# yukiteruono/pbsim3

Measured on AMD Instinct MI355X. Metric: simulated bases/sec, higher is better.
Workload: dtype u8

## Files before the change

### pbsim3_amd/csrc/ctx.h

```cpp
#pragma once
#include <hip/hip_runtime.h>
#include <limits.h>
#include <stdio.h>
#include <stdlib.h>
#include <stdint.h>

#include <algorithm>
#include <condition_variable>
#include <functional>
#include <memory>
#include <mutex>
#include <string>
#include <vector>

#include "../../include/pbsim3_amd.h"
#include "host_tables.h"
#include "kernels.h"

namespace pbsim {
extern thread_local std::string g_err;
int fail(const std::string &m);
}


// ... 33 lines not shown
  }
  template <class T>
  T *as() const {
    return reinterpret_cast<T *>(p);
  }
};

struct HostBuf {
  void *p = nullptr;
  size_t bytes = 0;
  ~HostBuf() {
    if (p) (void)hipHostFree(p);
  }
  hipError_t ensure(size_t n) {
    if (n <= bytes) return hipSuccess;
    if (p) (void)hipHostFree(p);
    p = nullptr;
    bytes = 0;
    size_t want = std::max<size_t>(n + n / 8 + 4096, 1u << 20);
    hipError_t e = hipHostMalloc(&p, want, hipHostMallocDefault);
    if (e != hipSuccess) {
      p = nullptr;
      return e;
    }
    bytes = want;
    return hipSuccess;
  }
};

using namespace pbsim;

constexpr int kMaxSlots = 6;
constexpr int kPipelineDepth = 2;
static_assert(kPipelineDepth >= 1 && kPipelineDepth <= kMaxSlots, "the pipeline's slots are the first of kMaxSlots");

constexpr size_t kScratchSlack = 64u << 10;
constexpr double kSinkBatchBases = 5.0e9;

constexpr int kDfBuffers = 5;
struct DfLane {
  DevBuf d_df_status, d_df_ctl;
  uint32_t epoch = 0;
  DevBuf d_df_dense[kDfBuffers];
  DevBuf d_df_code;
  HostBuf h_df_total, h_df_out[kDfBuffers];
  hipStream_t stream = nullptr;
  hipStream_t copy_stream = nullptr;
  bool own_streams = false;
  hipStream_t own[2] = {nullptr, nullptr};
  bool pre_valid = false, pre_own_staging = false, pre_elsewhere = false;
  const uint8_t *pre_text = nullptr;
  int64_t pre_n = 0;
  int pre_count = 0;
  hipStream_t lane_stream = nullptr;
  hipEvent_t ev_pre = nullptr;
  hipEvent_t ev_hand = nullptr;
  bool hand_open = false;
  hipEvent_t ev_df[kDfBuffers] = {}, ev_cp[kDfBuffers] = {};
  hipEvent_t ev_k0[kDfBuffers] = {}, ev_k1[kDfBuffers] = {};
  std::vector<std::unique_ptr<HostBuf>> arena_blocks;
  std::vector<size_t> arena_fill;
  std::vector<char> arena_touched;
  std::vector<int> arena_idle;
  std::vector<std::pair<const char *, int64_t>> arena_segs;
  size_t arena_bytes() const {
    size_t n = 0;
    for (const auto &b : arena_blocks) n += b->bytes;
    return n;
  }
  void arena_reset() {
    std::fill(arena_fill.begin(), arena_fill.end(), 0);
    arena_segs.clear();
  }
  char *arena_reserve(int64_t n, size_t max_bytes) {
    static const size_t kBlock = getenv("PBSIM_PINNED_BLOCK_KB") && atoll(getenv("PBSIM_PINNED_BLOCK_KB")) > 0
                                     ? (size_t)atoll(getenv("PBSIM_PINNED_BLOCK_KB")) << 10 : (size_t)256u << 20;
    const size_t need = ((size_t)n + 63) & ~(size_t)63;
    for (size_t i = 0; i < arena_blocks.size(); i++) {
      HostBuf &b = *arena_blocks[i];
      if (arena_fill[i] + need <= b.bytes) {
        char *p = (char *)b.p + arena_fill[i];
        arena_fill[i] += need;
        arena_touched[i] = 1;
        arena_segs.emplace_back(p, n);
        return p;
      }
    }
    const size_t want = std::max(kBlock, need);
    if (max_bytes && arena_bytes() + want > max_bytes) return nullptr;
    if (getenv("PBSIM_TRACE")) fprintf(stderr, "[pbsim arena] new block of %zu MB (lane holds %zu MB in %zu blocks)\n", want >> 20, arena_bytes() >> 20, arena_blocks.size());
    arena_blocks.emplace_back(new HostBuf);
    arena_fill.push_back(0);
    arena_touched.push_back(1);
    arena_idle.push_back(0);
    if (arena_blocks.back()->ensure(want) != hipSuccess) {
      arena_blocks.pop_back();
      arena_fill.pop_back();
      arena_touched.pop_back();
      arena_idle.pop_back();
      return nullptr;
    }
    arena_fill.back() = need;
    arena_segs.emplace_back((char *)arena_blocks.back()->p, n);
    return (char *)arena_blocks.back()->p;
  }
  static constexpr int kArenaIdleJobs = 16;
// ... 236 lines not shown
```

### pbsim3_amd/csrc/deflate_host.cpp

```cpp
#include <hip/hip_runtime.h>
#include <limits.h>
#include <math.h>
#include <stdio.h>
#include <stdlib.h>
#include <string.h>

#include <algorithm>
#include <chrono>
#include <functional>
#include <memory>
#include <string>
#include <thread>
#include <vector>

#include "ctx.h"
#include "engine_internal.h"
#include "unit_io.h"

extern "C" {

extern "C++" {
namespace {

int ensure_deflate_tables(pbsim_ctx *c) {
  if (c->d_df_tables.p) return PBSIM_SUCCEEDED;
  std::vector<uint32_t> t(1024 + 256);
  deflate_host_tables(t.data(), t.data() + 1024);
  if (!upload(c->d_df_tables, t.data(), t.size() * 4, c->stream)) return PBSIM_FAILED;
  HIP_OK(hipStreamSynchronize(c->stream));
  return PBSIM_SUCCEEDED;
}

struct DfGeom {
  int64_t piece, max_ch, n_pieces;
  int ahead, nbuf;
  int64_t off(int64_t j) const { return j * piece; }
  int64_t len(int64_t j, int64_t n) const { return std::min(piece, n - off(j)); }
};
DfGeom df_geom(int64_t n) {
  constexpr int64_t piece_chunks = DF_PIECE_CHUNKS;
  constexpr int kDfAhead = 4;
  static_assert(kDfAhead >= 1 && kDfAhead <= kDfBuffers - 1, "ahead + 1 dense buffers are in use");
  DfGeom g;
  g.piece = piece_chunks * DF_CHUNK;
  g.max_ch = std::min<int64_t>(piece_chunks, (n + DF_CHUNK - 1) / DF_CHUNK);
  g.n_pieces = (n + g.piece - 1) / g.piece;
  g.ahead = kDfAhead;
  g.nbuf = g.ahead + 1;
  return g;
}

int df_launch_piece(pbsim_ctx *c, DfLane &sl, const DfGeom &g, const uint8_t *d_text, int64_t n, int64_t j, bool wait_buffer,
                    bool own_staging, unsigned long long *d_prof) {
  const int b = (int)(j % g.nbuf);
  const int64_t off = g.off(j), len = g.len(j, n);
  const uint32_t *tab = c->d_df_tables.as<uint32_t>();
  int64_t *h_total = reinterpret_cast<int64_t *>(sl.h_df_total.p);
  HIP_OK(sl.d_df_dense[b].ensure((size_t)g.max_ch * DF_SLOT + 64, true));
  if (own_staging) HIP_OK(sl.h_df_out[b].ensure((size_t)g.max_ch * DF_SLOT + 64));
  if (wait_buffer) HIP_OK(hipStreamWaitEvent(sl.stream, sl.ev_cp[b], 0));
  uint8_t *dense = sl.d_df_dense[b].as<uint8_t>();
  if (((sl.epoch + 1) & 0x3fffffffu) == 0) {
    HIP_OK(hipMemsetAsync(sl.d_df_status.p, 0, sl.d_df_status.bytes, sl.stream));
    sl.epoch++;
  }
  launch_deflate(d_text + off, len, sl.d_df_status.as<uint64_t>(), sl.d_df_ctl.p, ++sl.epoch, dense, tab, tab + 1024,
                 sl.d_df_code.p, sl.stream, d_prof, sl.ev_k0[b], sl.ev_k1[b]);
  HIP_OK(hipGetLastError());
  HIP_OK(hipMemcpyAsync(&h_total[2 * b], sl.d_df_ctl.p, DF_CTL_BYTES, hipMemcpyDeviceToHost, sl.stream));
  HIP_OK(hipEventRecord(sl.ev_df[b], sl.stream));
  return PBSIM_SUCCEEDED;
}

int df_begin(pbsim_ctx *c, DfLane &sl, const uint8_t *d_text, int64_t n, bool own_staging, hipStream_t launch_stream) {
  if (!ensure_deflate_tables(c)) return PBSIM_FAILED;
  const DfGeom g = df_geom(n);
  const size_t status_bytes_was = sl.d_df_status.bytes;
  HIP_OK(sl.d_df_status.ensure((size_t)(g.piece / DF_CHUNK) * 8));
  HIP_OK(sl.d_df_ctl.ensure(DF_CTL_BYTES));
  HIP_OK(sl.h_df_total.ensure(DF_CTL_BYTES * kDfBuffers));
  HIP_OK(sl.d_df_code.ensure(DF_TABLE_BYTES + 288 * 4));
  int lane_index = 0;
  for (Slot &slot : c->slots)
    if (&slot.df[1] == &sl) lane_index = 1;
  hipStream_t lane_streams[2];
  if (sl.own_streams) {
    for (int i = 0; i < 2; i++)
      if (!sl.own[i]) HIP_OK(hipStreamCreateWithFlags(&sl.own[i], hipStreamNonBlocking));
    lane_streams[0] = sl.own[0];
    lane_streams[1] = sl.own[1];
  } else {
    for (int i = 0; i < 2; i++)
      if (!c->df_streams[lane_index][i]) HIP_OK(hipStreamCreateWithFlags(&c->df_streams[lane_index][i], hipStreamNonBlocking));
    lane_streams[0] = c->df_streams[lane_index][0];
    lane_streams[1] = c->df_streams[lane_index][1];
  }
  sl.lane_stream = lane_streams[0];
  sl.stream = launch_stream ? launch_stream : lane_streams[0];
  sl.copy_stream = lane_streams[1];
  if (sl.d_df_status.bytes != status_bytes_was) HIP_OK(hipMemsetAsync(sl.d_df_status.p, 0, sl.d_df_status.bytes, sl.stream));
  launch_deflate_table(d_text, n, reinterpret_cast<uint32_t *>(sl.d_df_code.as<uint8_t>() + DF_TABLE_BYTES), sl.d_df_code.p, sl.stream);
  if (!sl.ev_df[0]) {
    for (int i = 0; i < kDfBuffers; i++) {
      HIP_OK(hipEventCreateWithFlags(&sl.ev_df[i], hipEventDisableTiming));
      HIP_OK(hipEventCreateWithFlags(&sl.ev_cp[i], hipEventDisableTiming));
      HIP_OK(hipEventCreate(&sl.ev_k0[i]));
      HIP_OK(hipEventCreate(&sl.ev_k1[i]));
    }
  }
  unsigned long long *d_prof = nullptr;
  if (getenv("PBSIM_DEFLATE_PROF")) {
    HIP_OK(c->d_df_prof.ensure(128));
    HIP_OK(hipMemsetAsync(c->d_df_prof.p, 0, 128, sl.stream));
    d_prof = c->d_df_prof.as<unsigned long long>();
  }
  const int64_t first = std::min<int64_t>(launch_stream ? 1 : g.ahead, g.n_pieces);
  for (int64_t j = 0; j < first; j++)
    if (!df_launch_piece(c, sl, g, d_text, n, j, false, own_staging, d_prof)) return PBSIM_FAILED;
  sl.pre_count = (int)first;
  sl.pre_text = d_text;
  sl.pre_n = n;
  sl.pre_own_staging = own_staging;
  sl.pre_valid = true;
  sl.pre_elsewhere = launch_stream != nullptr;
  if (launch_stream) {
    if (!sl.ev_pre) HIP_OK(hipEventCreateWithFlags(&sl.ev_pre, hipEventDisableTiming));
    HIP_OK(hipEventRecord(sl.ev_pre, launch_stream));
  }
  return PBSIM_SUCCEEDED;
}

template <class F>
int deflate_stream(pbsim_ctx *c, DfLane &sl, const uint8_t *d_text, int64_t n, F &&consume,
                   const std::function<char *(int64_t)> *place = nullptr, const std::function<bool()> *tail_hook = nullptr) {
  if (n <= 0) return PBSIM_SUCCEEDED;
  const bool prelaunched = sl.pre_valid && sl.pre_text == d_text && sl.pre_n == n && sl.pre_own_staging == (place == nullptr);
  sl.pre_valid = false;
  const bool handed = prelaunched && sl.hand_open;
  if (!prelaunched && !pbsim::deflate_settle(sl)) return PBSIM_FAILED;
  if (!prelaunched && !df_begin(c, sl, d_text, n, place == nullptr, nullptr)) return PBSIM_FAILED;
  sl.pre_valid = false;
  if (handed && getenv("PBSIM_TRACE"))
    fprintf(stderr, "[deflate] lane call of %.1f MB found its head handed off (%d pieces launched behind the call in front)\n", n / 1e6,
            sl.pre_count);
  if (sl.pre_elsewhere) {
    sl.stream = sl.lane_stream;
    HIP_OK(hipStreamWaitEvent(sl.stream, sl.ev_pre, 0));
    sl.pre_elsewhere = false;
  }
  const DfGeom g = df_geom(n);
  const int64_t n_pieces = g.n_pieces;
  const int ahead = g.ahead, nbuf = g.nbuf;
  unsigned long long *d_prof = getenv("PBSIM_DEFLATE_PROF") ? c->d_df_prof.as<unsigned long long>() : nullptr;
  const bool trace = getenv("PBSIM_DEFLATE_TRACE") != nullptr;
  const auto now = []() { return std::chrono::duration<double, std::milli>(std::chrono::steady_clock::now().time_since_epoch()).count(); };
  double t_kernel = 0, t_copy = 0, t_consume = 0, t_begin = now();
  double t_first_copy = 0, t_last_copy = 0;
  bool hook_due = false;
  auto offer_tail = [&]() {
    if (tail_hook && hook_due && (*tail_hook)()) hook_due = false;
  };
  int64_t out_bytes = 0;
  std::vector<std::pair<hipEvent_t, hipEvent_t>> tev;
  bool used[kDfBuffers] = {false};
  int64_t *h_total = reinterpret_cast<int64_t *>(sl.h_df_total.p);
  auto launch = [&](int64_t j) -> int {
    return df_launch_piece(c, sl, g, d_text, n, j, used[(int)(j % nbuf)], place == nullptr, d_prof);
  };
  for (int64_t j = sl.pre_count; j < std::min<int64_t>(ahead, n_pieces); j++)
    if (!launch(j)) return PBSIM_FAILED;
  hook_due = n_pieces <= ahead;
  offer_tail();
  const char *prev_ptr = nullptr;
  int64_t prev_bytes = 0;
  int prev_buf = 0;
  for (int64_t k = 0; k < n_pieces; k++) {
    const int b = (int)(k % nbuf);
    const double t0 = now();
    HIP_OK(hipEventSynchronize(sl.ev_df[b]));
    t_kernel += now() - t0;
    const int64_t total = h_total[2 * b + 1];
    if ((uint64_t)h_total[2 * b] >> 32) return fail("deflate: a workgroup's look-back gave up waiting for its predecessors");
    out_bytes += total;
    {
      float ms = 0;
      if (hipEventElapsedTime(&ms, sl.ev_k0[b], sl.ev_k1[b]) == hipSuccess) {
        std::lock_guard<std::mutex> lk(c->prof_mu);
        c->prof_deflate_ms += ms;
        c->prof_deflate_launches++;
        c->prof_deflate_in += g.len(k, n);
        c->prof_deflate_out += total;
      }
    }
    char *dst = place ? (*place)(total) : (char *)sl.h_df_out[b].p;
    if (!dst) return fail("deflate: no room for a compressed piece");
    HIP_OK(hipStreamWaitEvent(sl.copy_stream, sl.ev_df[b], 0));
    if (trace) {
      hipEvent_t e0 = nullptr, e1 = nullptr;
      HIP_OK(hipEventCreate(&e0));
      HIP_OK(hipEventCreate(&e1));
      tev.emplace_back(e0, e1);
      HIP_OK(hipEventRecord(e0, sl.copy_stream));
    }
    if (k == 0) t_first_copy = now();
    HIP_OK(hipMemcpyAsync(dst, sl.d_df_dense[b].p, (size_t)total, hipMemcpyDeviceToHost, sl.copy_stream));
    if (trace) HIP_OK(hipEventRecord(tev.back().second, sl.copy_stream));
    HIP_OK(hipEventRecord(sl.ev_cp[b], sl.copy_stream));
    used[b] = true;
    if (prev_bytes) {
      const double t1 = now();
      HIP_OK(hipEventSynchronize(sl.ev_cp[prev_buf]));
      const double t2 = now();
      if (!consume(prev_ptr, prev_bytes)) return PBSIM_FAILED;
      t_copy += t2 - t1;
      t_consume += now() - t2;
    }
    prev_ptr = dst;
    prev_bytes = total;
    prev_buf = b;
    if (k + ahead < n_pieces && !launch(k + ahead)) return PBSIM_FAILED;
    if (k + ahead == n_pieces - 1) hook_due = true;
    offer_tail();
  }
  if (prev_bytes) {
    const double t1 = now();
    HIP_OK(hipEventSynchronize(sl.ev_cp[prev_buf]));
    const double t2 = now();
    t_last_copy = t2;
    if (!consume(prev_ptr, prev_bytes)) return PBSIM_FAILED;
    t_copy += t2 - t1;
    t_consume += now() - t2;
  }
  sl.hand_open = false;
  if (trace) {
    double t_link = 0, t_span = 0;
    float ms = 0;
    for (auto &e : tev) {
      if (hipEventElapsedTime(&ms, e.first, e.second) == hipSuccess) t_link += ms;
    }
    if (!tev.empty() && hipEventElapsedTime(&ms, tev.front().first, tev.back().second) == hipSuccess) t_span = ms;
    for (auto &e : tev) {
      (void)hipEventDestroy(e.first);
      (void)hipEventDestroy(e.second);
    }
    fprintf(stderr,
            "[deflate] %.1f MB -> %.1f MB in %.1f ms: waited %.1f ms for kernels, %.1f ms for copies, %.1f ms in the consumer; copies: "
            "%.1f ms on the engine within a span of %.1f ms (%.1f GB/s while copying); first copy enqueued at %.3f, last copy "
            "complete at %.3f ms%s%s\n",
            n / 1e6, out_bytes / 1e6, now() - t_begin, t_kernel, t_copy, t_consume, t_link, t_span, t_link > 0 ? out_bytes / t_link / 1e6 : 0.0,
            t_first_copy, t_last_copy, sl.own_streams ? " (chain lane)" : "", handed ? " (head handed off)" : "");
  }
  if (d_prof) {
    unsigned long long t[16];
    HIP_OK(hipMemcpy(t, d_prof, 128, hipMemcpyDeviceToHost));
    const double nch = (double)((n + DF_CHUNK - 1) / DF_CHUNK);
    static const char *names[7] = {"stage", "crc", "sizes+scan", "header", "tokens", "trailer", "store"};
    fprintf(stderr, "[deflate prof] %.0f chunks; us per chunk (lane 0):", nch);
    for (int i = 0; i < 7; ++i) fprintf(stderr, " %s %.1f", names[i], t[i] / nch / 100);
    fprintf(stderr, "\n");
  }
  return PBSIM_SUCCEEDED;
}

int deflate_to_host(pbsim_ctx *c, DfLane &sl, const uint8_t *d_text, int64_t n, char *host_dst, int64_t cap,
                    int64_t *out_bytes) {
  int64_t written = 0;
  const int ok = deflate_stream(c, sl, d_text, n, [&](const char *z, int64_t k) {
    if (written + k > cap) return fail("deflate: output buffer too small");
    memcpy(host_dst + written, z, (size_t)k);
    written += k;
    return PBSIM_SUCCEEDED;
  });
  *out_bytes = written;
  return ok;
}

}
}

extern "C++" int pbsim::deflate_pieces(pbsim_ctx *c, DfLane &lane, const uint8_t *d_text, int64_t n,
                                       const std::function<int(const char *, int64_t)> &consume,
                                       const std::function<char *(int64_t)> *place, const std::function<bool()> *tail_hook) {
  return deflate_stream(c, lane, d_text, n, consume, place, tail_hook);
}
extern "C++" int pbsim::deflate_handoff(pbsim_ctx *c, DfLane &next, int lane_index, const uint8_t *d_text, int64_t n,
                                        bool own_staging, hipEvent_t text_ready) {
  hipStream_t st = c->df_streams[lane_index][0];
  if (!st || next.own_streams || next.hand_open || n <= 0) return fail("deflate_handoff: bad argument");
  if (!next.ev_hand) HIP_OK(hipEventCreateWithFlags(&next.ev_hand, hipEventDisableTiming));
  HIP_OK(hipStreamWaitEvent(st, text_ready, 0));
  const int ok = df_begin(c, next, d_text, n, own_staging, nullptr);
  if (!ok) next.pre_valid = false;
  next.hand_open = true;
  HIP_OK(hipEventRecord(next.ev_hand, st));
  return ok;
}
extern "C++" int pbsim::deflate_settle(DfLane &lane) {
  if (!lane.hand_open) return PBSIM_SUCCEEDED;
  lane.pre_valid = false;
  HIP_OK(hipEventSynchronize(lane.ev_hand));
  lane.hand_open = false;
  return PBSIM_SUCCEEDED;
}
// ... 125 lines not shown
```

### pbsim3_amd/csrc/job.cpp

```cpp
#include <math.h>
#include <stdio.h>
#include <stdlib.h>
#include <string.h>

#include <algorithm>
#include <atomic>
#include <chrono>
#include <condition_variable>
#include <deque>
#include <future>
#include <mutex>
#include <thread>

#include "ctx.h"
#include "handoff.h"

using namespace pbsim;

namespace {

double now_us() {
  return std::chrono::duration<double, std::micro>(std::chrono::steady_clock::now().time_since_epoch()).count();
}

constexpr double kMinBatchBases = 2.0e9;
constexpr int kRoundsPerRecord = 4;

struct Rec {
  RefDesc ref;
  int64_t quota = 0, len_total = 0, next_read = 1, spec_read = 1;
  double spec_total = 0;
  int64_t cap = 0;
  bool bulk_done = false;
  bool done = false;
  int owner = -1;
  int tail_slot = -1;
  bool tail_waiting = false;
  int64_t read_off = 0, maf_off = 0;
  int64_t tail_read = 0, tail_maf = 0;
  StatsAcc st;
  bool merged = false;
};

struct Round {
  int rec, slot;
  int64_t first, n_per;
  double mean;
  bool clear;
};

struct Worker {
  std::thread th;
  std::mutex mu;
  std::condition_variable cv, cv_idle;
  std::deque<std::function<void()>> q;
  bool stop = false, running = false;
  int active = 0;
  struct Deferred {
    int key;
    std::function<bool()> ready;
    std::function<void()> run;
  };
  std::deque<Deferred> parked;
  int n_parked = 0;
  void defer(int key, std::function<bool()> ready, std::function<void()> run) {
    parked.push_back(Deferred{key, std::move(ready), std::move(run)});
    std::lock_guard<std::mutex> lk(mu);
    n_parked++;
  }
  bool run_parked() {
    bool any = false;
    for (size_t i = 0; i < parked.size();) {
      bool first_of_key = true;
      for (size_t j = 0; j < i; j++) first_of_key &= parked[j].key != parked[i].key;
      if (first_of_key && parked[i].ready()) {
        Deferred d = std::move(parked[i]);
        parked.erase(parked.begin() + (long)i);
        d.run();
        {
          std::lock_guard<std::mutex> lk(mu);
          n_parked--;
        }
        any = true;
        i = 0;
      } else {
        i++;
      }
    }
    return any;
  }
  void start(int device) {
    running = true;
    th = std::thread([this, device]() {
      (void)hipSetDevice(device);
      for (;;) {
        std::function<void()> f;
        {
          std::unique_lock<std::mutex> lk(mu);
          if (parked.empty()) cv.wait(lk, [&] { return stop || !q.empty(); });
          else cv.wait_for(lk, std::chrono::milliseconds(1), [&] { return stop || !q.empty(); });
          if (q.empty() && parked.empty()) return;
          if (!q.empty()) {
            f = std::move(q.front());
            q.pop_front();
            active++;
          }
        }
        if (f) {
          f();
          std::lock_guard<std::mutex> lk(mu);
          active--;
        }
        if (run_parked() || f) cv_idle.notify_all();
      }
    });
  }
  void post(std::function<void()> f) {
    {
      std::lock_guard<std::mutex> lk(mu);
      q.push_back(std::move(f));
    }
    cv.notify_one();
  }
  void drain() {
    if (!running) return;
    std::unique_lock<std::mutex> lk(mu);
    cv_idle.wait(lk, [&] { return q.empty() && active == 0 && n_parked == 0; });
  }
  void finish() {
    if (!running) return;
    drain();
    {
      std::lock_guard<std::mutex> lk(mu);
      stop = true;
    }
    cv.notify_all();
    th.join();
    running = false;
  }
  ~Worker() { finish(); }
};

struct Delivery {
  int slot = -1, rec = -1;
  bool mine = false;
  int64_t n_per = 0;
  std::shared_ptr<std::promise<int>> stage1;
  std::future<int> stage1_done;
  int64_t sizes[2] = {0, 0};
  int ok1 = PBSIM_SUCCEEDED;
  double t_wait0 = 0, t_wait1 = 0;
};

struct Job {
  pbsim_ctx *c;
  const pbsim_comm *comm;
  const pbsim_record_sink *sink;
  int rank = 0, W = 1;
  bool multi = false;
  std::vector<Rec> recs;
  std::deque<Round> fifo;
  double mean = 0;
  int depth = 3;
  int interleave = 1;
  int64_t reads_walked = 0, reads_delivered = 0, rounds = 0, bases = 0, ref_bases = 0, maf_columns = 0;
  double comm_us = 0;
  double bd_wait_walk = 0, bd_finalize = 0, bd_wait_bytes = 0, bd_account = 0, bd_tail_block = 0, bd_drain = 0, bd_slot_wait = 0,
         bd_merge = 0, bd_begin = 0, bd_tail_steps = 0;
  double bd_worker_busy = 0;
  int64_t n_topup = 0, n_tail_reads = 0, n_clear_missed = 0, n_exchanges = 0;
  bool trace = false;
  double t_start = 0;
  bool peer_failed = false;
  Worker worker;
  Worker tail_worker;
  std::mutex sink_mu[2];
  std::mutex out_mu;
  std::condition_variable out_cv;
  std::atomic<bool> delivering[kMaxSlots];
  std::atomic<bool> wfailed{false};
  std::mutex werr_mu;
  std::string werr;
  std::unique_ptr<Delivery> pending;
  std::unique_ptr<std::atomic<int>[]> rec_out;
  std::unique_ptr<std::atomic<int>[]> rec_bulk;
  std::unique_ptr<std::atomic<int>[]> rec_rounds_open;
  void round_closed(int rec) {
    --rec_rounds_open[(size_t)rec];
    { std::lock_guard<std::mutex> lk(out_mu); }
    out_cv.notify_all();
  }
  std::atomic<bool> giving_up{false};
  void wait_record(int rec) {
    std::unique_lock<std::mutex> lk(out_mu);
    out_cv.wait(lk, [&] { return rec_out[(size_t)rec].load() == 0; });
  }
  void delivered_one(std::atomic<int> *out, std::atomic<int> *bulk = nullptr) {
    --*out;
    if (bulk) --*bulk;
    { std::lock_guard<std::mutex> lk(out_mu); }
    out_cv.notify_all();
  }

  Job() {
    for (auto &d : delivering) d = false;
  }

  size_t n_collected = 0;
  bool seen11 = false;
  double bd_record_wait = 0;
  const DeviceFlags *record_arrived(int i) {
    JobRecord *jr = nullptr;
    {
      std::unique_lock<std::mutex> lk(c->job_mu);
      const double t0 = now_us();
      const bool came = c->job_cv.wait_for(lk, std::chrono::seconds(600),
                                           [&] { return c->job_records.size() > (size_t)i || c->job_feed_failed; });
      bd_record_wait += now_us() - t0;
      if (c->job_records.size() <= (size_t)i) {
        fail(!came ? "pbsim_job_run: a record announced by pbsim_job_expect did not arrive within 600 s" : c->job_feed_err);
        return nullptr;
      }
      jr = c->job_records[(size_t)i].get();
    }
    const double t1 = now_us();
// ... 242 lines not shown
  int arena_fill(Slot &sl, int64_t *read_gz, int64_t *maf_gz) {
    const pbsim_batch_info &bi = sl.b_info;
    *read_gz = *maf_gz = 0;
    return both_lanes(sl, [&](int which) -> int {
      DfLane &L = sl.df[which];
      L.arena_reset();
      const int64_t n = which == 0 ? bi.read_text_bytes : bi.maf_text_bytes;
      auto cb = which == 0 ? sink->on_read_text : sink->on_maf_text;
      if (!cb || n == 0) return PBSIM_SUCCEEDED;
      const uint8_t *d = which == 0 ? sl.d_read_text.as<uint8_t>() : sl.d_maf_text.as<uint8_t>();
      bool oom = false;
      const std::function<char *(int64_t)> place = [&](int64_t k) -> char * {
        char *p = L.arena_reserve(k, arena_max);
        if (!p) oom = true;
        return p;
      };
      const std::function<bool()> hook = tail_hook(which);
      if (!deflate_pieces(c, L, d, n, [](const char *, int64_t) { return PBSIM_SUCCEEDED; }, &place, handoff_on ? &hook : nullptr))
        return oom ? fail("out of pinned host memory for a compressed batch (PBSIM_PINNED_ARENA_MB bounds a lane's arena)") : PBSIM_FAILED;
      int64_t tot = 0;
      for (const auto &sg : L.arena_segs) tot += sg.second;
      (which == 0 ? *read_gz : *maf_gz) = tot;
      return PBSIM_SUCCEEDED;
    });
  }
  int arena_flush(Slot &sl, int64_t unit, int64_t read_at, int64_t maf_at) {
    return both_lanes(sl, [&](int which) -> int {
      int64_t at = which == 0 ? read_at : maf_at;
      for (const auto &sg : sl.df[which].arena_segs) {
        if (!call_sink(which, unit, sg.first, sg.second, at)) return fail(which == 0 ? "sink aborted (read text)" : "sink aborted (MAF text)");
        at += sg.second;
      }
      sl.df[which].arena_segs.clear();
      return PBSIM_SUCCEEDED;
    });
  }

  void submit_stage1(Delivery *d) {
    d->stage1 = std::make_shared<std::promise<int>>();
    d->stage1_done = d->stage1->get_future();
    if (!d->mine) {
      d->stage1->set_value(PBSIM_SUCCEEDED);
      return;
    }
    delivering[d->slot] = true;
    Slot *sl = &c->slots[d->slot];
    Rec *R = &recs[(size_t)d->rec];
    auto prom = d->stage1;
    int64_t *sizes = d->sizes;
    const int64_t read_at = R->read_off, maf_at = R->maf_off;
    std::atomic<int> *out = &rec_out[(size_t)d->rec], *bulk = &rec_bulk[(size_t)d->rec];
    ++*out;
    ++*bulk;
    worker.post([this, sl, R, prom, sizes, read_at, maf_at, out, bulk]() {
      const double w0 = now_us();
      int ok = PBSIM_SUCCEEDED;
      if (wants_text() && hipEventSynchronize(sl->ev_text) != hipSuccess) ok = fail("hipEventSynchronize failed (text emission)");
      if (!ok) {
      } else if (!wants_text()) {
        sizes[0] = sizes[1] = 0;
      } else if (!deflated()) {
        ok = fetch_plain(*sl);
        sizes[0] = sink->on_read_text ? sl->b_info.read_text_bytes : 0;
        sizes[1] = sink->on_maf_text ? sl->b_info.maf_text_bytes : 0;
      } else if (!multi) {
        ok = stream_deflated(*sl, R->ref.unit, read_at, maf_at, &sizes[0], &sizes[1]);
      } else {
        ok = arena_fill(*sl, &sizes[0], &sizes[1]);
      }
      if (!ok) worker_fail();
      bd_worker_busy += now_us() - w0;
      if (trace)
        fprintf(stderr, "[pbsim job r%d] t=%.1f ms   worker: bytes of rec %lld on their way for %.1f ms (%lld + %lld)\n", rank,
                (w0 - t_start) / 1e3, (long long)R->ref.unit, (now_us() - w0) / 1e3, (long long)sizes[0], (long long)sizes[1]);
      delivered_one(out, bulk);
      prom->set_value(ok);
    });
  }
  Slot *acct_slot = nullptr;
  Rec *acct_rec = nullptr;
  int account_deferred() {
    if (!acct_slot) return PBSIM_SUCCEEDED;
    Slot *sl = acct_slot;
    acct_slot = nullptr;
    const double t0 = now_us();
    const int ok = account_of(c, *sl, &acct_rec->st);
    bd_account += now_us() - t0;
    round_closed((int)(acct_rec - recs.data()));
    return ok;
  }
  int wait_pending(int64_t c3[3]) {
    c3[0] = c3[1] = c3[2] = 0;
    if (!pending) return PBSIM_SUCCEEDED;
    const double t0 = now_us();
    const int ok1 = pending->stage1_done.get();
    pending->ok1 = ok1;
    pending->t_wait0 = t0;
    pending->t_wait1 = now_us();
    bd_wait_bytes += pending->t_wait1 - t0;
    c3[0] = pending->mine ? pending->sizes[0] : 0;
    c3[1] = pending->mine ? pending->sizes[1] : 0;
    c3[2] = ok1 ? 0 : 1;
    return PBSIM_SUCCEEDED;
  }
  int apply_pending(const std::vector<int64_t> &S, int stride, int at, bool defer_account) {
    if (!pending) return PBSIM_SUCCEEDED;
    std::unique_ptr<Delivery> d = std::move(pending);
    Rec &R = recs[(size_t)d->rec];
    const int ok1 = d->ok1;
    int64_t read_at = R.read_off, maf_at = R.maf_off, read_all = 0, maf_all = 0, bad = 0;
    for (int q = 0; q < W; q++) {
      const int64_t *v = &S[(size_t)q * stride + at];
      if (q < rank) {
        read_at += v[0];
        maf_at += v[1];
      }
      read_all += v[0];
      maf_all += v[1];
      bad += v[2];
    }
    if (bad) {
      if (ok1) peer_failed = true;
      return ok1 ? fail("another rank of the job failed") : check_worker();
    }
    R.read_off += read_all;
    R.maf_off += maf_all;
    if (d->mine) {
      Slot *sl = &c->slots[d->slot];
      Rec *Rp = &R;
      const int slot = d->slot;
      const bool flush = deflated() && multi, plain = wants_text() && !deflated();
      acct_slot = sl;
      acct_rec = &R;
      std::atomic<int> *out = &rec_out[(size_t)d->rec], *bulk = &rec_bulk[(size_t)d->rec];
      if (flush || plain) {
        ++*out;
        ++*bulk;
      }
      if (!defer_account && !account_deferred()) return PBSIM_FAILED;
      if (flush || plain) {
        worker.post([this, sl, Rp, slot, flush, read_at, maf_at, out, bulk]() {
          const int ok = flush ? arena_flush(*sl, Rp->ref.unit, read_at, maf_at) : sink_plain(*sl, Rp->ref.unit, read_at, maf_at);
          if (!ok) worker_fail();
          delivering[slot] = false;
          delivered_one(out, bulk);
        });
      } else {
        delivering[slot] = false;
      }
    } else {
      round_closed(d->rec);
    }
    if (trace)
      fprintf(stderr, "[pbsim job r%d] t=%.1f ms rec %d delivery: waited %.1f ms for the bytes (%lld + %lld)\n", rank,
              (d->t_wait0 - t_start) / 1e3, d->rec + 1, (d->t_wait1 - d->t_wait0) / 1e3, (long long)d->sizes[0], (long long)d->sizes[1]);
    return check_worker();
  }
  int complete_pending(bool defer_account = false) {
    if (!account_deferred()) return PBSIM_FAILED;
    if (!pending) return PBSIM_SUCCEEDED;
    int64_t mine2[3];
    if (!wait_pending(mine2)) return PBSIM_FAILED;
// ... 121 lines not shown

  int finish_record(int rec) {
    Rec &R = recs[(size_t)rec];
    if (pending && pending->rec == rec && !complete_pending()) return PBSIM_FAILED;
    if (!account_deferred()) return PBSIM_FAILED;
    const double tt = now_us();
    int tail_ok = PBSIM_SUCCEEDED;
    std::string tail_err;
    if (rank == R.owner && !tail_poll(rec, true)) {
      tail_ok = PBSIM_FAILED;
      tail_err = g_err;
    }
    const double td = now_us();
    bd_tail_block += td - tt;
    wait_record(rec);
    bd_drain += now_us() - td;
    int64_t extra[3] = {R.tail_read, R.tail_maf, (tail_ok && !wfailed) ? 0 : 1};
    const double t0 = now_us();
    progress(4, rec);
    if (!stats_merge(&R.st, c->p, multi ? comm : nullptr, extra, 3)) return PBSIM_FAILED;
    bd_merge += now_us() - t0;
    if (!tail_ok) return fail(tail_err);
    if (!check_worker()) return PBSIM_FAILED;
    if (extra[2]) {
      peer_failed = true;
      return fail("another rank of the job failed");
    }
    R.merged = R.done = true;
    pbsim_stats st;
    stats_finish(R.st, c->p, R.ref.len, &st);
    c->st = R.st;
    c->st.blocks.clear();
    R.st = StatsAcc();
    if (sink && sink->on_record_done &&
        !sink->on_record_done(sink->user, recs[(size_t)rec].ref.unit, &st, R.read_off + extra[0], R.maf_off + extra[1]))
      return fail("sink aborted (record done)");
    return PBSIM_SUCCEEDED;
  }

  int begin_round(int rec) {
    Rec &R = recs[(size_t)rec];
    const double remaining = (double)R.quota - R.spec_total;
    int64_t n_total = (int64_t)(1.005 * remaining / mean) + 64;
    if (remaining <= 0) n_total = 64;
    int64_t n_per = std::min<int64_t>((n_total + W - 1) / W, R.cap);
    if (rounds < 2) n_per = std::min<int64_t>(n_per, std::max<int64_t>(64, (int64_t)((double)R.cap * (rounds == 0 ? 0.2 : 0.5))));
    n_per = std::max<int64_t>(n_per, 1);
    if (!collect(rec)) return PBSIM_FAILED;
    const int s = acquire_slot();
    c->cur = s;
    if (!settle_slot(s)) return PBSIM_FAILED;
    const double tb = now_us();
    if (trace) fprintf(stderr, "[pbsim job r%d] begin rec %d first=%lld n_per=%lld\n", rank, rec + 1, (long long)R.spec_read, (long long)n_per);
    if (!walk_begin(c, R.ref, R.spec_read + (int64_t)rank * n_per, n_per, -1)) return PBSIM_FAILED;
    bd_begin += now_us() - tb;
    const double after = R.spec_total + (double)W * (double)n_per * mean;
    const char *force_clear = getenv("PBSIM_JOB_CLEAR");
    const bool clear = force_clear ? atoi(force_clear) != 0
                                   : (double)R.quota - after > 0.04 * (double)W * (double)n_per * mean + 2.0 * (double)std::min<int64_t>(c->p.len_max, R.ref.len);
    fifo.push_back(Round{rec, s, R.spec_read, n_per, mean, clear});
    R.spec_read += (int64_t)W * n_per;
    R.spec_total += (double)W * (double)n_per * mean;
    reads_walked += n_per;
    rounds++;
    return PBSIM_SUCCEEDED;
  }

  static constexpr int kMsg = 8;
  int process_round() {
    const Round rd = fifo.front();
    fifo.pop_front();
    Rec &R = recs[(size_t)rd.rec];
    c->cur = rd.slot;
    struct Withdraw {
      Job *j;
      ~Withdraw() { (void)j->withdraw_next(); }
    } withdraw_at_exit{this};
    const double t0 = now_us();
    int64_t pass0 = 0, code = 0;
    std::string my_err;
    if (!pbsim_batch_walk_end(c, &pass0)) {
      my_err = g_err;
      code = (my_err.rfind("scratch budget exceeded", 0) == 0 && rd.n_per > 1) ? 1 : 2;
    }
    if (wfailed) code = 2;
    const double t1 = now_us();
    bd_wait_walk += t1 - t0;
    for (size_t r = 0; r < recs.size(); r++)
      if ((recs[r].tail_slot >= 0 || recs[r].tail_waiting) && !tail_poll((int)r, false)) return PBSIM_FAILED;
    c->cur = rd.slot;
    const int64_t max_raw = c->s().b_max_raw;
    pbsim_batch_info bi;
    memset(&bi, 0, sizeof bi);
    int fin_ok = PBSIM_SUCCEEDED;
    double t_fin = 0;
    std::vector<int64_t> A, B;
    int64_t msg[kMsg] = {pass0, code, max_raw, 0, 0, 0, 0, 0};
    bool c_applied = false;
    if (rd.clear) {
      if (code == 0) {
        const double tf = now_us();
        fin_ok = finalize_uncut(c, &bi) && finalize_text(c, &bi);
        if (!fin_ok) my_err = g_err;
        else publish_next(rd.slot);
        t_fin += now_us() - tf;
      }
      msg[3] = fin_ok ? 0 : 1;
      if (pending) {
        msg[4] = 1;
        if (!wait_pending(&msg[5])) return PBSIM_FAILED;
      }
      progress(6, rd.rec, rd.first, rd.n_per);
      if (!gather(msg, kMsg, &A)) return PBSIM_FAILED;
      c_applied = true;
    } else {
      progress(1, rd.rec, rd.first, rd.n_per);
      if (!gather(msg, kMsg, &A)) return PBSIM_FAILED;
    }
    int64_t worst = 0, pass0_sum = 0, before = R.len_total, raw_all = 0, bad_fin = 0;
    for (int q = 0; q < W; q++) {
      worst = std::max(worst, A[(size_t)q * kMsg + 1]);
      pass0_sum += A[(size_t)q * kMsg];
      raw_all = std::max(raw_all, A[(size_t)q * kMsg + 2]);
      bad_fin += A[(size_t)q * kMsg + 3];
      if (q < rank) before += A[(size_t)q * kMsg];
    }
    if (c_applied && worst != 2 && !apply_pending(A, kMsg, 5, true)) return PBSIM_FAILED;
    if (worst == 2 || (worst == 0 && bad_fin)) {
      drop_everything();
      if (wfailed) return check_worker();
      if (code != 2 && fin_ok) peer_failed = true;
      return fail(code == 2 || !fin_ok ? my_err : "another rank of the job failed");
    }
    if (worst == 1) {
      if (!complete_pending()) return PBSIM_FAILED;
      drop_everything(false);
      for (Rec &r : recs) {
        r.spec_read = r.next_read;
        r.spec_total = (double)r.len_total;
        r.cap = std::min(r.cap, std::max<int64_t>(1, rd.n_per / 2));
// ... 571 lines not shown
    const double mean_len = std::max(1.0, c->hdr.mean_len);
    const double want = (target / P / mean_len) * P * ((double)regions * (sf * mean_len + kScratchPad) * 1.12 + 64.0) * 1.08 + (64 << 20);
    const double share = std::min(48.0 * (1LL << 30), 0.14 * (double)(free_b + held));
    const int64_t auto_b = (int64_t)std::max(256.0 * (1 << 20), std::min(want, share));
    if ((double)auto_b > 1.10 * (double)c->scratch_budget || c->scratch_budget > 2 * auto_b) c->scratch_budget = auto_b;
  }
  if (const char *tr = getenv("PBSIM_JOB_TARGET_RANKS")) {
    std::vector<double> v;
    for (const char *q = tr; *q;) {
      char *e = nullptr;
      v.push_back(strtod(q, &e));
      if (e == q) break;
      q = *e == ',' ? e + 1 : e;
    }
    if (!v.empty() && v[(size_t)J.rank % v.size()] > 0) target = v[(size_t)J.rank % v.size()];
  }
  std::vector<int64_t> agree(n + 1);
  agree[0] = c->scratch_budget;
  J.progress(5, -1);
  if (multi) {
    if (!comm->all_reduce_i64(comm->user, agree.data(), 1, PBSIM_OP_MIN)) return fail("pbsim_comm.all_reduce_i64 failed");
    c->scratch_budget = agree[0];
  }
  J.mean = 0.97 * c->hdr.mean_len;
  for (size_t i = 0; i < n; i++) {
    Rec &R = J.recs[i];
    const double m = std::min<double>(c->hdr.mean_len, (double)R.ref.len);
    R.cap = std::max<int64_t>(1, std::min<int64_t>(batch_capacity_for(c, R.ref.len), (int64_t)(1.08 * target / P / m) + 64));
    agree[i + 1] = R.cap;
  }
  if (multi) {
    if (!comm->all_reduce_i64(comm->user, agree.data(), (int64_t)agree.size(), PBSIM_OP_MIN)) return fail("pbsim_comm.all_reduce_i64 failed");
    for (size_t i = 0; i < n; i++) J.recs[i].cap = agree[i + 1];
  }
  J.mean = std::min<double>(J.mean, (double)lens[0]);
  for (Slot &sl : c->slots) sl.b_enqueued = sl.b_walked = sl.b_finalized = false;
  {
    const char *am = getenv("PBSIM_PINNED_ARENA_MB");
    J.arena_max = (size_t)(am && atoll(am) > 0 ? atoll(am) : 16384) << 20;
  }
  int ready = (!J.deflated() || ensure_deflate_ready(c)) ? PBSIM_SUCCEEDED : PBSIM_FAILED;
  if (multi) {
    const std::string keep = g_err;
    int64_t bad = ready ? 0 : 1;
    if (!comm->all_reduce_i64(comm->user, &bad, 1, PBSIM_OP_MAX)) return fail("pbsim_comm.all_reduce_i64 failed");
    if (bad) {
      *settled = true;
      return ready ? fail("another rank of the job failed") : fail(keep);
    }
  } else if (!ready) {
    return PBSIM_FAILED;
  }
  const int keep_lds = c->walk_lds_kb;
  if (J.deflated()) c->walk_lds_kb = std::max(c->walk_lds_kb, 81);
  c->defer_text_sync = true;
  {
    const char *ho = getenv("PBSIM_JOB_HANDOFF");
    J.handoff_on = J.deflated() && c->deflate_parallel && !(ho && atoi(ho) == 0);
    const char *la = getenv("PBSIM_JOB_LOOKAHEAD");
    J.lookahead = delivers && !(la && atoi(la) == 0);
  }
  if (J.trace) fprintf(stderr, "[pbsim job r%d] entered at %.3f ms, round loop at %.3f ms\n", J.rank, J.t_start / 1e3, now_us() / 1e3);
  int ok = J.run();
  c->defer_text_sync = false;
  c->walk_lds_kb = keep_lds;
  for (Slot &sl : c->slots)
    if (sl.stream && hipStreamSynchronize(sl.stream) != hipSuccess && ok) ok = fail("hipStreamSynchronize failed at the end of the job");
  if (!ok) {
    const std::string keep = g_err;
    if (multi && !J.peer_failed && comm->abort) comm->abort(comm->user);
    *settled = true;
    J.drop_everything();
    J.worker.finish();
    J.tail_worker.finish();
    g_err = keep;
  }
  (void)J.withdraw_next();
  for (int s = 0; s < kMaxSlots; s++)
    if (!J.settle_slot(s) && ok) ok = PBSIM_FAILED;
  for (Slot &sl : c->slots)
    for (DfLane &L : sl.df) L.arena_trim();
  if (J.trace)
    fprintf(stderr, "[pbsim job r%d] returns at %.3f ms; hand-off %s: %lld lane heads launched at a tail, %lld of them never delivered\n",
            J.rank, now_us() / 1e3, J.handoff_on ? "on" : "off", (long long)J.n_handed, (long long)J.n_handed_void);
  {
    const double wall = now_us() - J.t_start;
    double *b = c->job_breakdown;
    b[0] = wall;
    b[1] = J.bd_wait_walk;
    b[2] = J.bd_finalize;
    b[3] = J.bd_wait_bytes;
    b[4] = J.comm_us;
    b[5] = J.bd_account;
    b[6] = J.bd_tail_block;
    b[7] = J.bd_drain;
    b[8] = J.bd_slot_wait + J.bd_record_wait;
    b[9] = J.bd_merge;
    b[10] = J.bd_begin;
    b[11] = J.bd_tail_steps;
    b[12] = J.bd_worker_busy;
    b[13] = (double)J.n_topup;
    b[14] = (double)J.n_tail_reads;
    b[15] = (double)J.depth;
  }
  c->job_counters[0] = J.reads_walked;
  c->job_counters[1] = J.reads_delivered;
  c->job_counters[2] = J.rounds;
// ... 50 lines not shown
```

### pbsim3_amd/csrc/kernels.h

```cpp
#pragma once
#include <hip/hip_runtime.h>
#include <stdint.h>

#include "modes.h"

namespace pbsim {

constexpr int kWG = 256;
constexpr int kLenBuckets = 4096;
constexpr int kBinPad = 16;
constexpr int kLenShift = 8;
constexpr int kScratchPad = 64;
constexpr int kMaxClasses = 64;
constexpr int32_t kWaveTransposed = 1 << 30;
constexpr int kHpTile = 4096;

enum : uint32_t {
  kErrScratchOverflow = 1u,
  kErrScratchBudget = 2u,
};

struct DeviceFlags {
  uint32_t error;
  uint32_t high_bytes;
// ... 177 lines not shown
  int32_t is_qs;
  uint32_t unit;
  const int32_t *len, *off;
  const int32_t *out_len, *maf_len, *nsub, *nins, *ndel;
  const int32_t *task_of_slot;
  const int32_t *wave_cap;
  const int64_t *wave_off;
  const uint8_t *scratch;
  const int32_t *read_unit;
  const uint8_t *read_minus;
  int64_t *task_off;
  ReadArrays out;
};

void launch_prepare_reference(uint8_t *seq, uint8_t *hp, int flag_hp11, int64_t len, int64_t *tile_first, int64_t *tile_last,
                              int64_t *carry_start, int64_t *carry_next, int keep_first_case, DeviceFlags *flags,
                              hipStream_t s);
void launch_squeeze_lines(const uint8_t *lines, int64_t bytes, uint8_t *dst, int64_t *tile_tmp, int64_t *scan_tmp, int64_t *total,
                          hipStream_t s);
void launch_header_wgs(const HeaderArgs &a, hipStream_t s);
void launch_header_trans(const HeaderArgs &a, hipStream_t s);
void launch_task_sort(const SortArgs &a, hipStream_t s);
void launch_chain_prepare(const HeaderArgs &a, int k, int32_t pass_num, const int32_t *task_of_slot, int32_t *masked,
                          int64_t n_slots_max, ChainState *chain, hipStream_t s);
void launch_chain_update(int k, int32_t pass_num, const int32_t *out_len, ChainState *chain, hipStream_t s);
void launch_chain_init(ChainState *chain, int64_t remaining, hipStream_t s);
void launch_walk_errhmm(const WalkArgs &a, int64_t n_slots_max, uint32_t lds_bytes, bool fast_rv, bool hp_bits,
                        hipStream_t s, int min_lds_kb);
constexpr int kCoopMaxStates = 31;
constexpr int kCoopWaves = 8;
void launch_walk_errhmm_coop(const WalkArgs &a, int n_wg, uint32_t lds_bytes, bool hp_bits, hipStream_t s);
int walk_errhmm_coop_resident(uint32_t lds_bytes, bool hp_bits);
constexpr int kQCoopMaxStates = 63;
void launch_walk_qshmm_coop(const WalkArgs &a, int n_wg, uint32_t lds_bytes, hipStream_t s);
void launch_qshmm_coop_qsum(const WalkArgs &a, int64_t n_slots_max, hipStream_t s);
void launch_walk_qshmm(const WalkArgs &a, int64_t n_slots_max, uint32_t lds_bytes, bool fast_rv, bool hp_bits,
                       hipStream_t s, int min_lds_kb);
void launch_walk_sample(const SampleArgs &a, bool hp_bits, hipStream_t s);
void launch_sample_qsum(const SampleArgs &a, hipStream_t s);
void launch_exclusive_scan_i64(const int64_t *in, int64_t *out, int64_t n, int64_t *tmp, int64_t *total, hipStream_t s);
void launch_gather_pass0_scan(const int32_t *out_len, int64_t n_reads, int32_t pass_num, int64_t *cum, int64_t *tmp,
                              int64_t *total, hipStream_t s);
void launch_quota_cut(const int64_t *cum, const int32_t *rawlen, int64_t n_reads, int64_t len_total_before,
                      int64_t quota, int force_all, DeviceFlags *flags, hipStream_t s);
void launch_cigar_count(const TextArgs &a, int64_t n_slots_max, const DeviceFlags *flags, hipStream_t s);
void launch_text_sizes(const TextArgs &a, DeviceFlags *flags, hipStream_t s);
void launch_text_emit(const TextArgs &a, int64_t n_slots_max, const DeviceFlags *flags, hipStream_t s);
void launch_export_sizes(const ExportArgs &a, DeviceFlags *flags, int64_t *scan_tmp, hipStream_t s);
void launch_export(const ExportArgs &a, int64_t n_slots_max, const DeviceFlags *flags, hipStream_t s);

#define DF_CHUNK 32768
#define DF_SLOT (DF_CHUNK + 64)
#define DF_PIECE_CHUNKS 8192
#define DF_SAMPLE_CHUNKS 64
#define DF_TABLE_HDR_DW 96
#define DF_TABLE_BYTES 2048
void deflate_host_tables(uint32_t *crc_table , uint32_t *pow128 );
void launch_deflate_table(const uint8_t *text, int64_t n_bytes, uint32_t *hist, void *table, hipStream_t s);
#define DF_CTL_BYTES 16
void launch_deflate(const uint8_t *text, int64_t n_bytes, uint64_t *status, void *ctl, uint32_t epoch, uint8_t *dense,
                    const uint32_t *d_crc_table, const uint32_t *d_pow128, const void *table, hipStream_t s,
                    unsigned long long *d_prof = nullptr ,
                    hipEvent_t ev_begin = nullptr, hipEvent_t ev_chunks_done = nullptr );

struct InflateMember {
  int64_t in_off, out_off;
  int32_t in_len, out_len;
  uint32_t crc, pad;
};
enum InflateStatus : int32_t {
  kInfOk = 0,
  kInfBlockType,
  kInfStoredLen,
  kInfTooMany,
  kInfClSet,
  kInfRepeat,
  kInfNoEob,
  kInfLitSet,
  kInfDistSet,
  kInfLitCode,
  kInfDistCode,
  kInfTooFar,
  kInfTruncated,
  kInfTrailing,
  kInfCrc,
  kInfLength,
  kInfCount
};
const char *inflate_reason(int32_t status);
void launch_inflate(const uint8_t *in, const InflateMember *members, int64_t n_members, uint8_t *out, int32_t *status,
                    const uint32_t *d_crc_table, const uint32_t *d_pow128, hipStream_t s);

constexpr int kSpTile = 1024;
inline int64_t sp_tiles(int64_t b0, int64_t b1) { return b1 > b0 ? (b1 - (b0 & ~(int64_t)(kSpTile - 1)) + kSpTile - 1) / kSpTile : 0; }
void launch_sp_count(const uint8_t *buf, int64_t b0, int64_t b1, int64_t *tile_count, int32_t *nul, hipStream_t s);
void launch_sp_lines(const uint8_t *buf, int64_t b0, int64_t b1, int phase, const int64_t *tile_base, uint32_t *rec_start,
                     uint32_t *rec_end, hipStream_t s);
void launch_sp_sums(const uint8_t *buf, const uint32_t *rec_start, const uint32_t *rec_end, int64_t n_rec, int32_t len_min,
                    int32_t len_max, double acc_min, double acc_max, const double *qprob , int32_t *rec_len,
                    double *accuracy, int64_t *padded, hipStream_t s);
void launch_sp_pool(const uint8_t *buf, const uint32_t *rec_start, const int32_t *rec_len, const int64_t *padded, const int64_t *off,
                    int64_t n_rec, uint8_t *pool, hipStream_t s);

enum : int32_t { kSbCounted = 0, kSbSkipped = 1, kSbNoQual = 2 };
void launch_sb_sums(const uint8_t *buf, const uint64_t *rec, int64_t n_rec, int32_t len_min, int32_t len_max, double acc_min, double acc_max,
                    const double *qprob , uint32_t *qual_at, int32_t *rec_len, int32_t *status, double *accuracy,
// ... 6 lines not shown
```

Measured before the change: 58.57 billion.

## Choose walk LDS size per round from measured delivery backlog

When output is deflated, the job no longer pins every walk launch to the large LDS request. It now measures walk time per read under each LDS setting, plus delivery bytes, link rate and text-emit time. Before each walk it asks whether the reads queued ahead would take longer to deliver than this walk takes, and uses the small, unthrottled LDS size only when they would not. Deflate piece size can now be overridden by an environment variable, but the default stays the same. The aim is to let the walk run at full occupancy when delivery is not the bottleneck, at the cost of measurement overhead and the risk that a wrong choice makes the walk contend with deflate.

```diff
diff --git a/pbsim3_amd/csrc/ctx.h b/pbsim3_amd/csrc/ctx.h
--- a/pbsim3_amd/csrc/ctx.h
+++ b/pbsim3_amd/csrc/ctx.h
@@ -109,6 +109,7 @@
   const uint8_t *pre_text = nullptr;
   int64_t pre_n = 0;
   int pre_count = 0;
+  int64_t piece_chunks = 0;
   hipStream_t lane_stream = nullptr;
   hipEvent_t ev_pre = nullptr;
   hipEvent_t ev_hand = nullptr;
diff --git a/pbsim3_amd/csrc/deflate_host.cpp b/pbsim3_amd/csrc/deflate_host.cpp
--- a/pbsim3_amd/csrc/deflate_host.cpp
+++ b/pbsim3_amd/csrc/deflate_host.cpp
@@ -14,6 +14,7 @@
 #include <vector>
 
 #include "ctx.h"
+#include "delivery_rules.h"
 #include "engine_internal.h"
 #include "unit_io.h"
 
@@ -37,8 +38,14 @@
   int64_t off(int64_t j) const { return j * piece; }
   int64_t len(int64_t j, int64_t n) const { return std::min(piece, n - off(j)); }
 };
-DfGeom df_geom(int64_t n) {
-  constexpr int64_t piece_chunks = DF_PIECE_CHUNKS;
+static_assert(pbsim::kDfChunkBytes == DF_CHUNK && pbsim::kDfPieceChunks == DF_PIECE_CHUNKS && pbsim::kDfPieceChunksMax == DF_PIECE_CHUNKS_MAX,
+              "delivery_rules.h restates the piece sizes of kernels.h");
+static_assert((uint64_t)DF_PIECE_CHUNKS_MAX * (DF_CHUNK + 31) < (1ull << 32), "the look-back adds a piece's member sizes in 32 bits");
+int64_t df_call_piece_chunks(int64_t n) {
+  const char *f = getenv("PBSIM_DEFLATE_PIECE_CHUNKS");
+  return pbsim::df_piece_chunks(n, f ? atoll(f) : 0);
+}
+DfGeom df_geom(int64_t n, int64_t piece_chunks) {
   constexpr int kDfAhead = 4;
   static_assert(kDfAhead >= 1 && kDfAhead <= kDfBuffers - 1, "ahead + 1 dense buffers are in use");
   DfGeom g;
@@ -74,7 +81,8 @@
 
 int df_begin(pbsim_ctx *c, DfLane &sl, const uint8_t *d_text, int64_t n, bool own_staging, hipStream_t launch_stream) {
   if (!ensure_deflate_tables(c)) return PBSIM_FAILED;
-  const DfGeom g = df_geom(n);
+  sl.piece_chunks = df_call_piece_chunks(n);
+  const DfGeom g = df_geom(n, sl.piece_chunks);
   const size_t status_bytes_was = sl.d_df_status.bytes;
   HIP_OK(sl.d_df_status.ensure((size_t)(g.piece / DF_CHUNK) * 8));
   HIP_OK(sl.d_df_ctl.ensure(DF_CTL_BYTES));
@@ -148,7 +156,7 @@
     HIP_OK(hipStreamWaitEvent(sl.stream, sl.ev_pre, 0));
     sl.pre_elsewhere = false;
   }
-  const DfGeom g = df_geom(n);
+  const DfGeom g = df_geom(n, sl.piece_chunks);
   const int64_t n_pieces = g.n_pieces;
   const int ahead = g.ahead, nbuf = g.nbuf;
   unsigned long long *d_prof = getenv("PBSIM_DEFLATE_PROF") ? c->d_df_prof.as<unsigned long long>() : nullptr;
@@ -246,9 +254,9 @@
     fprintf(stderr,
             "[deflate] %.1f MB -> %.1f MB in %.1f ms: waited %.1f ms for kernels, %.1f ms for copies, %.1f ms in the consumer; copies: "
             "%.1f ms on the engine within a span of %.1f ms (%.1f GB/s while copying); first copy enqueued at %.3f, last copy "
-            "complete at %.3f ms%s%s\n",
+            "complete at %.3f ms%s%s; %lld pieces of %lld chunks\n",
             n / 1e6, out_bytes / 1e6, now() - t_begin, t_kernel, t_copy, t_consume, t_link, t_span, t_link > 0 ? out_bytes / t_link / 1e6 : 0.0,
-            t_first_copy, t_last_copy, sl.own_streams ? " (chain lane)" : "", handed ? " (head handed off)" : "");
+            t_first_copy, t_last_copy, sl.own_streams ? " (chain lane)" : "", handed ? " (head handed off)" : "", (long long)n_pieces, (long long)sl.piece_chunks);
   }
   if (d_prof) {
     unsigned long long t[16];
diff --git a/pbsim3_amd/csrc/delivery_rules.h b/pbsim3_amd/csrc/delivery_rules.h
--- /dev/null
+++ b/pbsim3_amd/csrc/delivery_rules.h
@@ -0,0 +1,31 @@
+#pragma once
+#include <stdint.h>
+
+namespace pbsim {
+
+constexpr int64_t kDfChunkBytes = 32768;
+constexpr int64_t kDfPieceChunks = 8192;
+constexpr int64_t kDfPieceChunksMax = 65536;
+inline int64_t df_piece_chunks(int64_t n_bytes, int64_t forced) {
+  (void)n_bytes;
+  if (forced > 0) return forced < kDfPieceChunksMax ? forced : kDfPieceChunksMax;
+  return kDfPieceChunks;
+}
+
+struct WalkMeasure {
+  double bytes_per_read = 0;
+  double bytes_per_ms = 0;
+  double free_ms_per_read = 0;
+  double throttled_ms_per_read = 0;
+  double emit_ms_per_read = 0;
+};
+constexpr double kThrottledOverFree = 1.7;
+inline bool walk_throttled(int64_t reads_in_front, int64_t n_reads, const WalkMeasure &m) {
+  if (reads_in_front <= 0) return false;
+  const double walk = m.throttled_ms_per_read > 0 ? m.throttled_ms_per_read : kThrottledOverFree * m.free_ms_per_read;
+  if (!(m.bytes_per_read > 0 && m.bytes_per_ms > 0 && walk > 0 && m.emit_ms_per_read > 0)) return true;
+  const double in_front_ms = (double)reads_in_front * m.bytes_per_read / m.bytes_per_ms;
+  return in_front_ms > (walk + m.emit_ms_per_read) * (double)n_reads;
+}
+
+}
diff --git a/pbsim3_amd/csrc/job.cpp b/pbsim3_amd/csrc/job.cpp
--- a/pbsim3_amd/csrc/job.cpp
+++ b/pbsim3_amd/csrc/job.cpp
@@ -13,6 +13,7 @@
 #include <thread>
 
 #include "ctx.h"
+#include "delivery_rules.h"
 #include "handoff.h"
 
 using namespace pbsim;
@@ -46,6 +47,7 @@
   int rec, slot;
   int64_t first, n_per;
   double mean;
+  bool throttled;
   bool clear;
 };
 
@@ -150,6 +152,7 @@
   int64_t sizes[2] = {0, 0};
   int ok1 = PBSIM_SUCCEEDED;
   double t_wait0 = 0, t_wait1 = 0;
+  double link_ms = 0, emit_ms = 0;
 };
 
 struct Job {
@@ -171,6 +174,32 @@
   int64_t n_topup = 0, n_tail_reads = 0, n_clear_missed = 0, n_exchanges = 0;
   bool trace = false;
   double t_start = 0;
+  bool walk_choice = false;
+  int walk_force = -1;
+  int walk_free_kb = 27, walk_throttled_kb = 81;
+  WalkMeasure wm;
+  int64_t wm_walk_reads[2] = {0, 0}, wm_link_bytes = 0;
+  void note_walk(bool throttled, int64_t n_reads, double ms) {
+    if (ms <= 0 || n_reads <= 0 || 2 * n_reads < wm_walk_reads[throttled]) return;
+    wm_walk_reads[throttled] = std::max(wm_walk_reads[throttled], n_reads);
+    (throttled ? wm.throttled_ms_per_read : wm.free_ms_per_read) = ms / (double)n_reads;
+  }
+  void note_delivery(const Delivery &d) {
+    const int64_t bytes = d.sizes[0] + d.sizes[1];
+    if (bytes <= 0 || d.n_per <= 0 || d.link_ms <= 0 || 2 * bytes < wm_link_bytes) return;
+    wm_link_bytes = std::max(wm_link_bytes, bytes);
+    wm.bytes_per_read = (double)bytes / (double)d.n_per;
+    wm.bytes_per_ms = (double)bytes / d.link_ms;
+    if (d.emit_ms > 0) wm.emit_ms_per_read = d.emit_ms / (double)d.n_per;
+  }
+  int64_t reads_in_front() {
+    int64_t n = 0;
+    if (pending && pending->mine && pending->stage1_done.valid() &&
+        pending->stage1_done.wait_for(std::chrono::seconds(0)) != std::future_status::ready)
+      n += pending->n_per;
+    for (const Round &r : fifo) n += r.n_per;
+    return n;
+  }
   bool peer_failed = false;
   Worker worker;
   Worker tail_worker;
@@ -519,10 +548,13 @@
     std::atomic<int> *out = &rec_out[(size_t)d->rec], *bulk = &rec_bulk[(size_t)d->rec];
     ++*out;
     ++*bulk;
-    worker.post([this, sl, R, prom, sizes, read_at, maf_at, out, bulk]() {
+    worker.post([this, d, sl, R, prom, sizes, read_at, maf_at, out, bulk]() {
       const double w0 = now_us();
       int ok = PBSIM_SUCCEEDED;
       if (wants_text() && hipEventSynchronize(sl->ev_text) != hipSuccess) ok = fail("hipEventSynchronize failed (text emission)");
+      const double w1 = now_us();
+      float emit_ms = 0;
+      if (ok && walk_choice && hipEventElapsedTime(&emit_ms, sl->ev_t0, sl->ev_t1) == hipSuccess) d->emit_ms = emit_ms;
       if (!ok) {
       } else if (!wants_text()) {
         sizes[0] = sizes[1] = 0;
@@ -536,6 +568,7 @@
         ok = arena_fill(*sl, &sizes[0], &sizes[1]);
       }
       if (!ok) worker_fail();
+      d->link_ms = (now_us() - w1) / 1e3;
       bd_worker_busy += now_us() - w0;
       if (trace)
         fprintf(stderr, "[pbsim job r%d] t=%.1f ms   worker: bytes of rec %lld on their way for %.1f ms (%lld + %lld)\n", rank,
@@ -575,6 +608,7 @@
     std::unique_ptr<Delivery> d = std::move(pending);
     Rec &R = recs[(size_t)d->rec];
     const int ok1 = d->ok1;
+    if (walk_choice && d->mine && ok1) note_delivery(*d);
     int64_t read_at = R.read_off, maf_at = R.maf_off, read_all = 0, maf_all = 0, bad = 0;
     for (int q = 0; q < W; q++) {
       const int64_t *v = &S[(size_t)q * stride + at];
@@ -802,13 +836,26 @@
     if (!settle_slot(s)) return PBSIM_FAILED;
     const double tb = now_us();
     if (trace) fprintf(stderr, "[pbsim job r%d] begin rec %d first=%lld n_per=%lld\n", rank, rec + 1, (long long)R.spec_read, (long long)n_per);
-    if (!walk_begin(c, R.ref, R.spec_read + (int64_t)rank * n_per, n_per, -1)) return PBSIM_FAILED;
+    const int64_t in_front = walk_choice ? reads_in_front() : 0;
+    const bool throttled = walk_choice && (walk_force >= 0 ? walk_force != 0 : walk_throttled(in_front, n_per, wm));
+    const int keep_kb = c->walk_lds_kb;
+    if (walk_choice) c->walk_lds_kb = throttled ? walk_throttled_kb : walk_free_kb;
+    if (trace && walk_choice)
+      fprintf(stderr,
+              "[pbsim job r%d] walk of rec %d first=%lld: %d KB of LDS asked for (%s%s): %lld reads in front, %.0f B/read at %.1f MB/ms; "
+              "per 1000 reads walk %.3f | %.3f ms (free | throttled), text %.3f ms\n",
+              rank, rec + 1, (long long)R.spec_read, c->walk_lds_kb, throttled ? "throttled" : "free", walk_force >= 0 ? ", forced" : "",
+              (long long)in_front, wm.bytes_per_read, wm.bytes_per_ms / 1e6, 1e3 * wm.free_ms_per_read, 1e3 * wm.throttled_ms_per_read,
+              1e3 * wm.emit_ms_per_read);
+    const int began = walk_begin(c, R.ref, R.spec_read + (int64_t)rank * n_per, n_per, -1);
+    c->walk_lds_kb = keep_kb;
+    if (!began) return PBSIM_FAILED;
     bd_begin += now_us() - tb;
     const double after = R.spec_total + (double)W * (double)n_per * mean;
     const char *force_clear = getenv("PBSIM_JOB_CLEAR");
     const bool clear = force_clear ? atoi(force_clear) != 0
                                    : (double)R.quota - after > 0.04 * (double)W * (double)n_per * mean + 2.0 * (double)std::min<int64_t>(c->p.len_max, R.ref.len);
-    fifo.push_back(Round{rec, s, R.spec_read, n_per, mean, clear});
+    fifo.push_back(Round{rec, s, R.spec_read, n_per, mean, throttled, clear});
     R.spec_read += (int64_t)W * n_per;
     R.spec_total += (double)W * (double)n_per * mean;
     reads_walked += n_per;
@@ -836,6 +883,10 @@
     if (wfailed) code = 2;
     const double t1 = now_us();
     bd_wait_walk += t1 - t0;
+    if (walk_choice && code == 0) {
+      float walk_ms = 0;
+      if (hipEventElapsedTime(&walk_ms, c->s().ev1, c->s().ev2) == hipSuccess) note_walk(rd.throttled, rd.n_per, walk_ms);
+    }
     for (size_t r = 0; r < recs.size(); r++)
       if ((recs[r].tail_slot >= 0 || recs[r].tail_waiting) && !tail_poll((int)r, false)) return PBSIM_FAILED;
     c->cur = rd.slot;
@@ -1513,7 +1564,13 @@
     return PBSIM_FAILED;
   }
   const int keep_lds = c->walk_lds_kb;
-  if (J.deflated()) c->walk_lds_kb = std::max(c->walk_lds_kb, 81);
+  if (J.deflated()) {
+    J.walk_choice = true;
+    J.walk_free_kb = keep_lds;
+    J.walk_throttled_kb = c->walk_lds_kb = std::max(c->walk_lds_kb, 81);
+    const char *wt = getenv("PBSIM_JOB_WALK_THROTTLE");
+    if (wt && *wt) J.walk_force = atoi(wt) != 0;
+  }
   c->defer_text_sync = true;
   {
     const char *ho = getenv("PBSIM_JOB_HANDOFF");
diff --git a/pbsim3_amd/csrc/kernels.h b/pbsim3_amd/csrc/kernels.h
--- a/pbsim3_amd/csrc/kernels.h
+++ b/pbsim3_amd/csrc/kernels.h
@@ -253,6 +253,7 @@
 #define DF_CHUNK 32768
 #define DF_SLOT (DF_CHUNK + 64)
 #define DF_PIECE_CHUNKS 8192
+#define DF_PIECE_CHUNKS_MAX 65536
 #define DF_SAMPLE_CHUNKS 64
 #define DF_TABLE_HDR_DW 96
 #define DF_TABLE_BYTES 2048
```

Result: no change. 58.32 billion (-0.4%).
